# guanjq/targetdiff

Measured on NVIDIA H100. Metric: molecules/sec (1000-step sampling, CrossDocked pocket shape), higher is better.
Workload: dtype f32 (storage, LayerNorm, softmax, accumulation); GEMM operands as 2-piece bf16 splits on wgmma (3 products, ~16-bit operand mantissa)

## Files before the change

### targetdiff_b200/csrc/engine.cu

```cuda
#include <math.h>
#include <stdarg.h>
#include <stdio.h>
#include <stdlib.h>
#include <string.h>

#include <list>
#include <map>
#include <string>
#include <vector>

#include "../../include/tdiff.h"
#include "sampler.cuh"
#include "tdiff_common.cuh"

static thread_local char g_err[1024] = "";
static int set_err(int code, const char* fmt, ...) {
  va_list ap;
  va_start(ap, fmt);
  vsnprintf(g_err, sizeof(g_err), fmt, ap);
  va_end(ap);
  return code;
}
#define CK(call)                                                                                       \
  do {                                                                                                 \
// ... 36 lines not shown
  unsigned char* img_arena = nullptr;
  int mlp_mode = 2;
  bool mlp_v4 = true;
  std::vector<TdLayer> layers;
  const float *w_prot = nullptr, *b_prot = nullptr, *wl_t = nullptr, *bl = nullptr;
  const float *ew_w1t = nullptr, *ew_b1 = nullptr, *ew_g = nullptr, *ew_b = nullptr, *ew_w2 = nullptr, *ew_off = nullptr;
  float ew_b2 = 0.f, ew_coeff = -0.5f;
  int num_blocks = 1, ew_mode = 0 , out_fc = 0, time_emb = 0;
  int num_x2h = 1, num_h2x = 1, sync_twoup = 0;
  const float* w_time = nullptr;
  const float* zeros128 = nullptr;
  DevBuf ew_x2h, ew_h2x, hagg, time_norm;
  DevBuf h_sync;
  const float *hd_w1t = nullptr, *hd_b1 = nullptr, *hd_w2 = nullptr, *hd_b2 = nullptr;
  const float *t_c0 = nullptr, *t_ct = nullptr, *t_logvar = nullptr, *t_la = nullptr, *t_l1ma = nullptr, *t_lca = nullptr, *t_l1mca = nullptr,
              *t_sra = nullptr, *t_srm1 = nullptr;
  bool bound = false, has_ligand = false, have_graph = false;
  bool restrict_last = false;
  bool knn_incremental = false;
  bool have_prev = false;
  bool env_no_fused_agg = false, env_no_restrict = false, env_no_graph = false, env_knn_full = false, env_no_slot_keep = false;
  int B = 0, N = 0, Np = 0, Nl = 0, K = 0, max_ng = 0, final_buf = 0;
  int KQ = 0, hybrid = 0;
  DevBuf node_ptr, prot_ptr, prot_node, prot_graph, lig_node, lig_graph, node_lig;
  DevBuf rel_flag, rel_list, n_rel, work_list, n_work, knn_cache;
  DevBuf x2h_rows, lig_rows, rel_rows, rel_counts;
  long long x2h_n_dst = 0, x2h_split = 0, lig_n_dst = 0;
  int row_pad = 4;
  int free_depth = 0;
  int env_free_depth = 2;
  bool free_ready = false;
  DevBuf h_free, dirty, free_rows, free_counts, lig_save;
  long long free_stride = 0;
  DevBuf xm0, xm1, offset, h0, h, P, q, src, src_prev, etype, e_w, dist, kbuf, vbuf, v16, lig_pos, lig_v, logits;
  DevBuf step, err_flag, node_off, total_edges;
  DevBuf stage[8];
  cudaStream_t own_stream = nullptr;
  cudaEvent_t ev_fork = nullptr, ev_join = nullptr;
  long long launches = 0;
  bool profiling = false;
  std::vector<EvPair> events;
  double ms_acc[EV_KINDS] = {0, 0, 0, 0};
  long long n_acc[EV_KINDS] = {0, 0, 0, 0};
};

namespace {
struct Packer {
  std::map<std::string, const tdiff_tensor*> byname;
  std::vector<float> host;
  std::vector<unsigned char> img;
  std::string missing;
  std::list<std::vector<float>> keep;
  const float* get(const std::string& name, int64_t numel) {
    auto it = byname.find(name);
    if (it == byname.end() || it->second->numel != numel || it->second->data == nullptr) {
      if (missing.empty()) missing = name + (it == byname.end() ? " (absent)" : " (wrong size)");
      return nullptr;
    }
    return it->second->data;
  }
  size_t alloc(size_t n) {
    size_t off = (host.size() + 63) / 64 * 64;
    host.resize(off + n, 0.0f);
    return off;
  }
};
// ... 387 lines not shown
      const SubOff& so = is_h2x ? sh[l][idx - num_x2h] : sx[l][idx];
      sl.wn_t = A + so.wn_t; sl.bn = A + so.bn; sl.wn_img = IM ? IM + so.wn_img : nullptr;
      sl.k = mk_mlp(A, IM, so.k, 0, 256); sl.v = mk_mlp(A, IM, so.v, 128, 384); sl.q = mk_mlp(A, IM, so.q, 512, 512);
      sl.ew_w = so.ew_w >= 0 ? A + so.ew_w : nullptr; sl.ew_b = so.ew_b;
      sl.out_wa_img = so.out_wa >= 0 ? IM + so.out_wa : nullptr; sl.out_wb_img = so.out_wb >= 0 ? IM + so.out_wb : nullptr;
      sl.out_b1 = so.out_b1 >= 0 ? A + so.out_b1 : nullptr;
      memset(&sl.out, 0, sizeof(sl.out));
      if (so.out_w2 >= 0) {
        sl.out.w2_img = IM + so.out_w2; sl.out.ln_g = A + so.out_g; sl.out.ln_b = A + so.out_b; sl.out.b2 = A + so.out_b2; sl.out.nout = TD_H;
      }
    }
  }
  if (e->step.ensure(sizeof(int)) || e->err_flag.ensure(sizeof(int)) || e->total_edges.ensure(sizeof(long long))) {
    tdiff_destroy(e); return set_err(TDIFF_ECUDA, "cudaMalloc failed");
  }
  cudaMemset(e->err_flag.p, 0, sizeof(int));
  if (cudaStreamCreateWithFlags(&e->own_stream, cudaStreamNonBlocking) != cudaSuccess ||
      cudaEventCreateWithFlags(&e->ev_fork, cudaEventDisableTiming) != cudaSuccess ||
      cudaEventCreateWithFlags(&e->ev_join, cudaEventDisableTiming) != cudaSuccess) {
    tdiff_destroy(e); return set_err(TDIFF_ECUDA, "stream/event creation failed");
  }
  *out = e;
  return TDIFF_OK;
}

extern "C" void tdiff_destroy(tdiff_engine* e) {
  if (!e) return;
  cudaSetDevice(e->device);
  for (auto& ev : e->events) { cudaEventDestroy(ev.a); cudaEventDestroy(ev.b); }
  if (e->own_stream) cudaStreamDestroy(e->own_stream);
  if (e->ev_fork) cudaEventDestroy(e->ev_fork);
  if (e->ev_join) cudaEventDestroy(e->ev_join);
  DevBuf* bufs[] = {&e->node_ptr, &e->prot_ptr, &e->prot_node, &e->prot_graph, &e->lig_node, &e->lig_graph, &e->node_lig, &e->xm0, &e->xm1,
                    &e->rel_flag, &e->rel_list, &e->n_rel, &e->work_list, &e->n_work, &e->knn_cache, &e->x2h_rows, &e->lig_rows, &e->rel_rows, &e->rel_counts, &e->ew_x2h, &e->ew_h2x, &e->h_sync, &e->hagg, &e->time_norm, &e->h_free, &e->dirty, &e->free_rows, &e->free_counts, &e->lig_save, &e->offset, &e->h0, &e->h, &e->P, &e->q, &e->src, &e->src_prev, &e->etype, &e->e_w, &e->dist, &e->kbuf, &e->vbuf, &e->v16, &e->lig_pos,
                    &e->lig_v, &e->logits, &e->step, &e->err_flag, &e->node_off, &e->total_edges};
  for (auto* b : bufs) b->release();
  for (auto& b : e->stage) b.release();
  if (e->arena) cudaFree(e->arena);
  if (e->img_arena) cudaFree(e->img_arena);
  delete e;
}

extern "C" int tdiff_bind_batch(tdiff_engine* e, int B, const int32_t* pc, const int32_t* lc, const float* d_ppos, const float* d_pfeat,
                                int center_mode, void* stream) {
  if (!e || !pc || !lc || B < 1) return set_err(TDIFF_EINVAL, "bind_batch: bad arguments");
  if (center_mode != 0 && center_mode != 1) return set_err(TDIFF_EINVAL, "center_mode %d (0 'none' | 1 'protein')", center_mode);
  cudaStream_t st = (cudaStream_t)stream;
  CK(cudaSetDevice(e->device));
  long long N = 0, Np = 0, Nl = 0;
  int max_ng = 0;
  for (int g = 0; g < B; ++g) {
    if (pc[g] < 0 || lc[g] < 0) return set_err(TDIFF_EINVAL, "negative atom count in graph %d", g);
    Np += pc[g]; Nl += lc[g];
    if (pc[g] + lc[g] > max_ng) max_ng = pc[g] + lc[g];
  }
  N = Np + Nl;
  if (N <= 0) return set_err(TDIFF_EINVAL, "empty batch");
  if (e->hybrid) {
    int max_lc = 0;
    for (int g = 0; g < B; ++g) {
      if (lc[g] > max_lc) max_lc = lc[g];
      if (lc[g] > 0 && pc[g] < e->KQ)
        return set_err(TDIFF_EINVAL, "cutoff_mode 'hybrid': graph %d has %d protein atoms < k = %d (torch.topk fails in the reference too)", g, pc[g], e->KQ);
    }
    const int need = e->KQ + (max_lc > 0 ? max_lc - 1 : 0);
    if (need > TD_KMAX)
      return set_err(TDIFF_EINVAL, "cutoff_mode 'hybrid': k + n_ligand - 1 = %d + %d - 1 exceeds the %d neighbour slots per node", e->KQ, max_lc, TD_KMAX);
// ... 18 lines not shown
  bad |= e->node_ptr.ensure((B + 1) * 4) | e->prot_ptr.ensure((B + 1) * 4) | e->prot_node.ensure(Np * 4 + 4) | e->prot_graph.ensure(Np * 4 + 4);
  bad |= e->lig_node.ensure(Nl * 4 + 4) | e->lig_graph.ensure(Nl * 4 + 4) | e->node_lig.ensure(N * 4);
  bad |= e->xm0.ensure(N * 16) | e->xm1.ensure(N * 16) | e->offset.ensure((size_t)B * 16);
  bad |= e->h0.ensure(N * TD_H * 4) | e->h.ensure(N * TD_H * 4) | e->P.ensure((size_t)(N + 1) * TD_NPROJ * 4) | e->q.ensure(N * TD_H * 4);
  bad |= e->src.ensure(slots * 4) | e->src_prev.ensure(slots * 4) | e->etype.ensure(slots) | e->e_w.ensure(slots * 4) | e->dist.ensure(slots * 4);
  const bool v4 = e->mlp_mode == 2 && e->mlp_v4;
  int gcd128 = 128;
  while (K % gcd128) gcd128 >>= 1;
  e->row_pad = 128 / gcd128;
  const long long pad = e->row_pad, nPpad = (Np + pad - 1) / pad * pad, nLpad = (Nl + pad - 1) / pad * pad;
  e->x2h_n_dst = nPpad + nLpad; e->x2h_split = nPpad; e->lig_n_dst = nLpad;
  std::vector<int> x2h_rows((size_t)(nPpad + nLpad), -1), lig_rows((size_t)nLpad, -1);
  for (long long i = 0; i < Np; ++i) x2h_rows[i] = prot_node[i];
  for (long long i = 0; i < Nl; ++i) { x2h_rows[nPpad + i] = lig_node[i]; lig_rows[i] = lig_node[i]; }
  if (v4) bad |= e->x2h_rows.ensure(x2h_rows.size() * 4 + 4) | e->lig_rows.ensure(lig_rows.size() * 4 + 4) | e->rel_rows.ensure(x2h_rows.size() * 4 + 4) |
                 e->rel_counts.ensure(16);
  const bool fuse = v4 && K == 32 && !e->env_no_fused_agg && e->ew_mode != 2;
  if (e->ew_mode == 1) bad |= e->ew_x2h.ensure(slots * 4) | e->ew_h2x.ensure(slots * 4);
  if (e->out_fc) bad |= e->hagg.ensure((size_t)N * TD_H * 4);
  if (e->sync_twoup && e->num_x2h > 0 && e->num_h2x > 0) bad |= e->h_sync.ensure((size_t)N * TD_H * 4);
  if (e->time_emb) bad |= e->time_norm.ensure((size_t)B * 4 + 16);
  bad |= e->kbuf.ensure(v4 ? (size_t)(nPpad + nLpad) * K * TD_HEADS * 4 + 64 : slots * TD_H * 4);
  if (!fuse) bad |= e->vbuf.ensure(slots * TD_H * 4);
  bad |= e->v16.ensure((size_t)nLpad * K * TD_HEADS * 4 + 16);
  int min_pc = 1 << 30;
  for (int g = 0; g < B; ++g) if (pc[g] < min_pc) min_pc = pc[g];
  e->free_ready = false;
  e->free_depth = (fuse && !e->hybrid && Nl > 0 && min_pc > K) ? e->env_free_depth : 0;
  const int x2h_evals = (int)e->layers.size() * e->num_x2h;
  if (e->free_depth > x2h_evals - 1) e->free_depth = x2h_evals - 1 > 0 ? x2h_evals - 1 : 0;
  if (e->free_depth > 0)
    bad |= e->h_free.ensure((size_t)e->free_depth * N * TD_H * 4) | e->dirty.ensure((size_t)e->free_depth * N + 16) |
           e->free_rows.ensure((size_t)e->free_depth * x2h_rows.size() * 4 + 4) | e->free_counts.ensure((size_t)e->free_depth * 16) |
           e->lig_save.ensure((size_t)Nl * 20 + 32);
  e->free_stride = (long long)x2h_rows.size();
  bad |= e->lig_pos.ensure(Nl * 16 + 16) | e->lig_v.ensure(Nl * 4 + 4) | e->logits.ensure((size_t)Nl * e->cfg.num_classes * 4 + 4);
  bad |= e->node_off.ensure(N * 8) | e->rel_flag.ensure(N + 16) | e->rel_list.ensure(N * 4 + 64) | e->n_rel.ensure(16) | e->work_list.ensure(N * 4 + 64) | e->n_work.ensure(16);
  e->knn_incremental = !e->env_knn_full && Np > 0;
  if (e->knn_incremental) bad |= e->knn_cache.ensure((size_t)N * (e->KQ + 1) * 8);
  if (bad) return set_err(TDIFF_ECUDA, "out of device memory binding a batch of %lld nodes (%zu edge slots)", N, slots);
  CK(cudaMemcpyAsync(e->node_ptr.p, node_ptr.data(), (B + 1) * 4, cudaMemcpyHostToDevice, st));
  CK(cudaMemcpyAsync(e->prot_ptr.p, prot_ptr.data(), (B + 1) * 4, cudaMemcpyHostToDevice, st));
  if (Np) {
    CK(cudaMemcpyAsync(e->prot_node.p, prot_node.data(), Np * 4, cudaMemcpyHostToDevice, st));
    CK(cudaMemcpyAsync(e->prot_graph.p, prot_graph.data(), Np * 4, cudaMemcpyHostToDevice, st));
  }
  if (Nl) {
    CK(cudaMemcpyAsync(e->lig_node.p, lig_node.data(), Nl * 4, cudaMemcpyHostToDevice, st));
    CK(cudaMemcpyAsync(e->lig_graph.p, lig_graph.data(), Nl * 4, cudaMemcpyHostToDevice, st));
  }
  CK(cudaMemcpyAsync(e->node_lig.p, node_lig.data(), N * 4, cudaMemcpyHostToDevice, st));
  if (v4) {
    if (!x2h_rows.empty()) CK(cudaMemcpyAsync(e->x2h_rows.p, x2h_rows.data(), x2h_rows.size() * 4, cudaMemcpyHostToDevice, st));
    if (!lig_rows.empty()) CK(cudaMemcpyAsync(e->lig_rows.p, lig_rows.data(), lig_rows.size() * 4, cudaMemcpyHostToDevice, st));
  }
  CK(cudaStreamSynchronize(st));
  CK(cudaMemsetAsync(e->offset.p, 0, (size_t)B * 16, st));
  if (e->time_emb) CK(cudaMemsetAsync(e->time_norm.p, 0, (size_t)B * 4, st));
  CK(cudaMemsetAsync(e->h0.p, 0, (size_t)N * TD_H * 4, st));
  CK(cudaMemsetAsync(e->xm0.p, 0, (size_t)N * 16, st));
  CK(cudaMemsetAsync(e->xm1.p, 0, (size_t)N * 16, st));
  CK(cudaMemsetAsync(e->etype.p, 0, slots, st));
  CK(cudaMemsetAsync(e->P.as<float>() + (size_t)N * TD_NPROJ, 0, (size_t)TD_NPROJ * 4, st));
  if (center_mode == 1) td_launch_segment_mean3(d_ppos, e->prot_ptr.as<int>(), B, e->offset.as<float4>(), st);
  td_launch_place_protein(d_ppos, e->prot_node.as<int>(), e->prot_graph.as<int>(), e->offset.as<float4>(), (int)Np, e->xm0.as<float4>(),
                          e->xm1.as<float4>(), st);
  td_launch_protein_embed(d_pfeat, (int)Np, e->cfg.protein_feat_dim, e->w_prot, e->b_prot, e->prot_node.as<int>(), e->h0.as<float>(), st);
  e->launches += 3;
  if (e->knn_incremental) {
    td_launch_knn_cache(e->xm0.as<float4>(), e->node_ptr.as<int>(), e->prot_ptr.as<int>(), B, max_ng, e->KQ, e->knn_cache.as<unsigned long long>(), st);
    e->launches += 1;
  }
  CK(cudaGetLastError());
  e->bound = true;
  return TDIFF_OK;
}

extern "C" int tdiff_set_ligand(tdiff_engine* e, const float* d_pos, const int64_t* d_v, int apply_center, void* stream) {
  if (!e || !e->bound) return set_err(TDIFF_ESTATE, "set_ligand before bind_batch");
  if (e->Nl > 0 && !d_pos) return set_err(TDIFF_EINVAL, "null ligand positions");
  if (!e->has_ligand && e->Nl > 0 && !d_v) return set_err(TDIFF_EINVAL, "ligand types required on first set_ligand");
  cudaStream_t st = (cudaStream_t)stream;
  CK(cudaSetDevice(e->device));
  td_launch_set_ligand(d_pos, (const long long*)d_v, e->lig_graph.as<int>(), e->offset.as<float4>(), apply_center, e->Nl,
                       e->cfg.num_classes, e->lig_pos.as<float4>(), e->lig_v.as<int>(), e->err_flag.as<int>(), st);
  e->launches += 1;
  if (d_v) {
    int flag = 0;
    CK(cudaMemcpyAsync(&flag, e->err_flag.p, sizeof(int), cudaMemcpyDeviceToHost, st));
    CK(cudaStreamSynchronize(st));
    if (flag) {
      cudaMemsetAsync(e->err_flag.p, 0, sizeof(int), st);
      e->has_ligand = false;
      return set_err(TDIFF_EINVAL, "ligand atom type index >= num_classes (%d)", e->cfg.num_classes);
    }
  }
// ... 29 lines not shown
  }
  ~Prof() { if (on) { cudaEventRecord(ev.b, st); e->events.push_back(ev); } }
};

enum RowList { ROWS_ALL = 0, ROWS_LIGAND = 1, ROWS_RELEVANT = 2 };
bool fused_logits(const tdiff_engine* e) { return e->mlp_mode == 2 && e->mlp_v4; }
void edge_mlp(tdiff_engine* e, const float* P, const float4* xm, const int* src, const unsigned char* etype, RowList list, int K, const TdMlp& m,
              const float* offsets, float coeff, float* out, cudaStream_t st, const float* e_w, const float* qnode = nullptr,
              const float* agg_logits = nullptr, float* agg_h = nullptr, int key_softmax = 0, int free_layer = -1) {
  if (fused_logits(e) && m.w2_img && m.tabcls_img) {
    const int* rows = list == ROWS_ALL ? e->x2h_rows.as<int>() : list == ROWS_LIGAND ? e->lig_rows.as<int>() : e->rel_rows.as<int>();
    const int* counts = list == ROWS_RELEVANT ? e->rel_counts.as<int>() : nullptr;
    if (free_layer >= 0) {
      rows = e->free_rows.as<int>() + (size_t)free_layer * e->free_stride;
      counts = e->free_counts.as<int>() + 4 * free_layer;
    }
    const long long n_dst = list == ROWS_LIGAND ? e->lig_n_dst : e->x2h_n_dst;
    const long long split = list == ROWS_LIGAND ? 0 : e->x2h_split;
    const int by_slot = (list != ROWS_LIGAND && !key_softmax && agg_logits == nullptr) ? 1 : 0;
    td_launch_edge_mlp_v4(P, e->N, src, etype, e->dist.as<float>(), rows, n_dst, split, counts, K, m,
                          e->host_arena.data() + (offsets - e->arena), coeff, e->host_arena.data() + (m.ln_b - e->arena),
                          e->host_arena.data() + (m.b2 - e->arena), qnode, out, by_slot, agg_logits, e_w, agg_h, key_softmax,
                          e->sm_count, st);
    return;
  }
  const int* row_nodes = list == ROWS_LIGAND ? e->lig_node.as<int>() : nullptr;
  const long long n_rows = (long long)(list == ROWS_LIGAND ? e->Nl : e->N) * K;
  if (e->mlp_mode != 0 && m.nout == TD_H && m.w2_img)
    td_launch_edge_mlp_tc(P, xm, src, etype, e->dist.as<float>(), row_nodes, n_rows, K, m, m.w2_img, e->mlp_mode, offsets, coeff, out, e->sm_count, st);
  else
    td_launch_edge_mlp(P, xm, src, etype, row_nodes, n_rows, K, m, offsets, coeff, out, e->sm_count, st);
}

void node_side(tdiff_engine* e, const float* h, int N, const TdSubLayer& sl, float* P, float* q, cudaStream_t st, const int* rows = nullptr,
               const int* d_n = nullptr) {
  if (fused_logits(e) && sl.wn_img && sl.q.w2_img) {
    td_launch_node_side_v4(h, N, sl.wn_img, sl.bn, sl.q, P, q, rows, d_n, e->sm_count, st);
  } else if (e->mlp_mode != 0 && sl.wn_img && sl.q.w2_img) {
    TdMlp pm = sl.q;
    pm.b2 = sl.bn;
    td_launch_rows_tc(1, h, TD_H, 0, N, pm, sl.wn_img, e->mlp_mode, P, TD_NPROJ, TD_NPROJ / TD_H, rows, d_n, e->sm_count, st);
    td_launch_rows_tc(2, P, TD_NPROJ, 512, N, sl.q, sl.q.w2_img, e->mlp_mode, q, TD_H, 1, rows, d_n, e->sm_count, st);
  } else {
    td_launch_node_proj(h, N, sl.wn_t, sl.bn, P, st);
    td_launch_node_q(P, N, sl.q, q, st);
  }
}

void run_forward(tdiff_engine* e, cudaStream_t st, int fix_x, int free_build = 0, float* blk_pos = nullptr, float* blk_logits = nullptr) {
  const int N = e->N, Nl = e->Nl, K = e->K;
  float4* xm[2] = {e->xm0.as<float4>(), e->xm1.as<float4>()};
  const int* src = e->src.as<int>();
  const unsigned char* etype = e->etype.as<unsigned char>();
  float* h = e->h.as<float>();
  float* P = e->P.as<float>();
  float* q = e->q.as<float>();
  td_launch_scatter_ligand_pos(e->lig_pos.as<float4>(), e->lig_node.as<int>(), Nl, xm[0], st);
  td_launch_init_h(e->h0.as<float>(), xm[0], e->lig_v.as<int>(), e->node_lig.as<int>(), e->wl_t, e->bl, e->w_time, e->time_norm.as<float>(),
                   e->lig_graph.as<int>(), N, h, st);
  e->launches += 2;
  int cur = 0;
  const int KC = e->cfg.num_classes;
  auto snapshot = [&](int i) {
    if (blk_pos) {
      td_launch_gather_xyz(xm[cur], e->lig_node.as<int>(), Nl, blk_pos + (size_t)i * Nl * 3, st);
      e->launches += 1;
    }
    if (blk_logits) {
      td_launch_head(h, e->lig_node.as<int>(), Nl, e->hd_w1t, e->hd_b1, e->hd_w2, e->hd_b2, KC, blk_logits + (size_t)i * Nl * KC, st);
      e->launches += 1;
    }
  };
  if (Nl > 0) snapshot(0);
  const int n_blocks = free_build ? 1 : e->num_blocks;
  for (int blk = 0; blk < n_blocks; ++blk) {
// ... 9 lines not shown
                         use_free ? e->dirty.as<unsigned char>() : nullptr, e->work_list.as<int>(), e->n_work.as<int>(), (e->ew_mode != 0 ? 1 : 0) | (e->env_no_slot_keep ? 2 : 0), st);
    e->have_prev = true;
    for (int l = 0; l < use_free; ++l) {
      unsigned char* dl = e->dirty.as<unsigned char>() + (size_t)l * N;
      if (l > 0) td_launch_dirty_propagate(dl - N, src, N, K, dl, st);
      td_launch_rel_rows(dl, xm[cur], N, e->lig_rows.as<int>(), (int)e->lig_n_dst, e->row_pad, e->free_rows.as<int>() + (size_t)l * e->free_stride,
                         e->free_counts.as<int>() + 4 * l, st);
      e->launches += l > 0 ? 3 : 2;
    }
    td_launch_rel_compact(e->rel_flag.as<unsigned char>(), N, e->rel_list.as<int>(), e->n_rel.as<int>(), st);
    e->launches += 4;
    if (fused_logits(e) && e->restrict_last && last_blk && e->num_x2h > 0) {
      td_launch_rel_rows(e->rel_flag.as<unsigned char>(), xm[cur], N, e->lig_rows.as<int>(), (int)e->lig_n_dst, e->row_pad, e->rel_rows.as<int>(),
                         e->rel_counts.as<int>(), st);
      e->launches += 2;
    }
    const float4* xm_blk = xm[cur];
    const int NX = e->num_x2h, NH = e->num_h2x;
    const size_t L = e->layers.size();
    int g = 0;
    for (size_t l = 0; l < L && !(free_build && g >= free_build); ++l) {
      const TdLayer& ly = e->layers[l];
      const float* ew_x = e->ew_mode == 1 ? e->ew_x2h.as<float>() : e->e_w.as<float>();
      const float* ew_h = e->ew_mode == 1 ? e->ew_h2x.as<float>() : e->e_w.as<float>();
      const bool run_h2x = !free_build && !fix_x && Nl > 0 && NH > 0;
      const float* h_h2x = h;
      if (e->sync_twoup && run_h2x && NX > 0) {
        cudaMemcpyAsync(e->h_sync.p, h, (size_t)N * TD_H * 4, cudaMemcpyDeviceToDevice, st);
        h_h2x = e->h_sync.as<float>();
      }
      for (int i = 0; i < NX && !(free_build && g >= free_build); ++i, ++g) {
        const TdSubLayer& sx = ly.x2h[i];
        const int fl = g < use_free ? g : -1;
        node_side(e, h, N, sx, P, q, st);
        if (e->mlp_mode != 0 && (i == 0 || e->ew_mode == 1)) {
          TdEwR ew = {nullptr, nullptr, 0.f, 0.f, ly.offsets, ly.coeff, nullptr, nullptr};
          if (e->ew_mode == 1) {
            const TdSubLayer& sh0 = NH > 0 ? ly.h2x[0] : sx;
            ew.w_x2h = sx.ew_w; ew.w_h2x = sh0.ew_w; ew.b_x2h = sx.ew_b; ew.b_h2x = sh0.ew_b; ew.out_x2h = e->ew_x2h.as<float>(); ew.out_h2x = e->ew_h2x.as<float>();
          }
          td_launch_edge_geom(xm[cur], src, etype, N, K, e->dist.as<float>(), ew, st);
          e->launches += 1;
        }
        const bool fuse_agg = fused_logits(e) && K == 32 && !e->env_no_fused_agg && e->ew_mode != 2;
        const bool sub = fuse_agg && e->restrict_last && last_blk && l + 1 == L && i + 1 == NX && !e->env_no_restrict && !e->out_fc;
        const RowList rl = sub ? ROWS_RELEVANT : ROWS_ALL;
        float* agg_target = h;
        if (e->out_fc) {
          agg_target = e->hagg.as<float>();
          cudaMemsetAsync(agg_target, 0, (size_t)N * TD_H * 4, st);
        }
        {
          Prof pr(e, st, EV_EDGE_MLP);
          edge_mlp(e, P, xm[cur], src, etype, rl, K, sx.k, ly.offsets, ly.coeff, e->kbuf.as<float>(), st, ew_x, fused_logits(e) ? q : nullptr, nullptr,
                   nullptr, fuse_agg ? 1 : 0, fl);
          edge_mlp(e, P, xm[cur], src, etype, rl, K, sx.v, ly.offsets, ly.coeff, e->vbuf.as<float>(), st, ew_x, nullptr,
                   fuse_agg ? e->kbuf.as<float>() : nullptr, fuse_agg ? agg_target : nullptr, 0, fl);
        }
        if (!fuse_agg) {
          Prof pr(e, st, EV_AGG_H);
          if (fused_logits(e))
            td_launch_aggregate_h_logits(e->kbuf.as<float>(), e->vbuf.as<float>(), ew_x, src, e->out_fc ? agg_target : h, agg_target, N, K,
                                         e->ew_mode == 2 ? sx.ew_w : nullptr, sx.ew_b, st);
          else td_launch_aggregate_h(e->kbuf.as<float>(), e->vbuf.as<float>(), e->e_w.as<float>(), src, q, h, h, N, K, st);
        }
        e->launches += fuse_agg ? 4 : 5;
        if (e->out_fc) {
          float* t1 = P;
          float* t2 = P + (size_t)N * TD_H;
          TdMlp m1 = sx.out;
          m1.b2 = e->zeros128;
          td_launch_rows_tc(1, agg_target, TD_H, 0, N, m1, sx.out_wa_img, e->mlp_mode, t1, TD_H, 1, nullptr, nullptr, e->sm_count, st);
          m1.b2 = sx.out_b1;
          td_launch_rows_tc(1, h, TD_H, 0, N, m1, sx.out_wb_img, e->mlp_mode, t2, TD_H, 1, nullptr, nullptr, e->sm_count, st);
          td_launch_add_rows(t1, t2, t1, (long long)N * TD_H, st);
          td_launch_rows_tc(2, t1, TD_H, 0, N, sx.out, sx.out.w2_img, e->mlp_mode, t2, TD_H, 1, nullptr, nullptr, e->sm_count, st);
          td_launch_add_rows(h, t2, h, (long long)N * TD_H, st);
          e->launches += 6;
        }
        if (fl >= 0) {
          td_launch_restore_clean(e->dirty.as<unsigned char>() + (size_t)fl * N, xm_blk, e->h_free.as<float>() + (size_t)fl * N * TD_H, N, h, st);
          e->launches += 1;
        }
        if (free_build) cudaMemcpyAsync(e->h_free.as<float>() + (size_t)g * N * TD_H, h, (size_t)N * TD_H * 4, cudaMemcpyDeviceToDevice, st);
      }
      if (!run_h2x) continue;
      for (int j = 0; j < NH; ++j) {
        const TdSubLayer& sh = ly.h2x[j];
        if (j > 0 || NX == 0) {
          td_launch_edge_geom_rows(xm[cur], src, etype, e->lig_node.as<int>(), Nl, K, e->dist.as<float>(), e->ew_mode == 1 ? sh.ew_w : nullptr, sh.ew_b,
                                   ly.offsets, ly.coeff, e->ew_h2x.as<float>(), st);
          e->launches += 1;
        }
        {
          const bool rel = fused_logits(e) && !e->env_no_restrict;
          node_side(e, h_h2x, N, sh, P, q, st, rel ? e->rel_list.as<int>() : nullptr, rel ? e->n_rel.as<int>() : nullptr);
        }
        {
          Prof pr(e, st, EV_EDGE_MLP);
          edge_mlp(e, P, xm[cur], src, etype, ROWS_LIGAND, K, sh.k, ly.offsets, ly.coeff, e->kbuf.as<float>(), st, ew_h, fused_logits(e) ? q : nullptr);
          edge_mlp(e, P, xm[cur], src, etype, ROWS_LIGAND, K, sh.v, ly.offsets, ly.coeff, e->v16.as<float>(), st, ew_h);
        }
        {
          Prof pr(e, st, EV_AGG_X);
          if (fused_logits(e))
            td_launch_aggregate_x_logits(e->kbuf.as<float>(), e->v16.as<float>(), ew_h, src, xm[cur], e->lig_node.as<int>(), xm[cur ^ 1], Nl, K, st);
          else
            td_launch_aggregate_x(e->kbuf.as<float>(), e->v16.as<float>(), e->e_w.as<float>(), src, q, xm[cur], e->lig_node.as<int>(), xm[cur ^ 1], Nl, K, st);
        }
        e->launches += 5;
        cur ^= 1;
      }
    }
    if (Nl > 0) snapshot(blk + 1);
  }
  if (free_build) return;
  td_launch_head(h, e->lig_node.as<int>(), Nl, e->hd_w1t, e->hd_b1, e->hd_w2, e->hd_b2, e->cfg.num_classes, e->logits.as<float>(), st);
  e->launches += 1;
  e->final_buf = cur;
  e->have_graph = true;
  e->have_prev = true;
}
}

extern "C" int tdiff_set_time(tdiff_engine* e, const float* d_time_norm, void* stream) {
  if (!e || !e->bound) return set_err(TDIFF_ESTATE, "set_time before bind_batch");
  if (!e->time_emb) return TDIFF_OK;
  if (!d_time_norm) return set_err(TDIFF_EINVAL, "null time array");
  CK(cudaSetDevice(e->device));
  CK(cudaMemcpyAsync(e->time_norm.p, d_time_norm, (size_t)e->B * 4, cudaMemcpyDeviceToDevice, (cudaStream_t)stream));
// ... 367 lines not shown
```

### targetdiff_b200/csrc/node_side.cu

```cuda
#include "tdiff_common.cuh"
#include "hopper_mma.cuh"

namespace ns {

constexpr int kWG = 3;
constexpr int kThreads = kWG * 128;
constexpr int kTile = 64;
constexpr int kAtom = 128 * 128;
constexpr int kPiece = 2 * kAtom;
constexpr int kBlock = 2 * kPiece;
constexpr int kImgStride = 3 * kPiece;
constexpr int kHBuf = kTile * TD_H * 4;
constexpr size_t kSmem = 1024 + 2 * kBlock + kWG * kHBuf + 4 * TD_H * sizeof(float);
static_assert(kSmem <= 227 * 1024, "shared-memory map");

__device__ __forceinline__ uint32_t smem_u32(const void* p) { return (uint32_t)__cvta_generic_to_shared(p); }
__device__ __forceinline__ uint32_t cvt_bf16x2(float hi, float lo) {
  uint32_t d;
  asm("cvt.rn.bf16x2.f32 %0, %1, %2;" : "=r"(d) : "f"(hi), "f"(lo));
  return d;
}
__device__ __forceinline__ void stg64(float* p, float a, float b) { asm volatile("st.global.v2.f32 [%0], {%1,%2};" ::"l"(p), "f"(a), "f"(b) : "memory"); }
__device__ __forceinline__ void fence_proxy_async() { asm volatile("fence.proxy.async.shared::cta;" ::: "memory"); }

__device__ __forceinline__ void stage_weights(unsigned char* sW, const unsigned char* w0, const unsigned char* w1, float* sPar,
                                              const float* p0, const float* p1, const float* p2, const float* p3) {
  for (int i = threadIdx.x; i < kBlock / 16; i += kThreads) {
    reinterpret_cast<uint4*>(sW)[i] = reinterpret_cast<const uint4*>(w0)[i];
    reinterpret_cast<uint4*>(sW + kBlock)[i] = reinterpret_cast<const uint4*>(w1)[i];
  }
  for (int i = threadIdx.x; i < TD_H; i += kThreads) {
    if (p0) sPar[i] = p0[i];
    if (p1) sPar[TD_H + i] = p1[i];
    if (p2) sPar[2 * TD_H + i] = p2[i];
    if (p3) sPar[3 * TD_H + i] = p3[i];
  }
  fence_proxy_async();
  __syncthreads();
}

struct Rows {
  const int* list;
  const int* d_n;
  long long n;
};

__device__ __forceinline__ uint32_t chunk_pos(int r, int c) { return (uint32_t)(r * 512 + ((c ^ ((r & 3) << 1)) << 4)); }
__device__ __forceinline__ void bar_sync_wg(int wg) { asm volatile("bar.sync %0, 128;" ::"r"(1 + wg) : "memory"); }

__device__ __forceinline__ void load_tile_async(uint32_t buf, const float* __restrict__ in, const Rows& rw, long long n, long long tile, int t) {
  const int l = t & 31;
#pragma unroll 1
  for (int r = t >> 5; r < kTile; r += 4) {
    const long long i = tile * kTile + r;
    const long long node = i < n ? (rw.list ? (long long)rw.list[i] : i) : 0;
    asm volatile("cp.async.cg.shared.global [%0], [%1], 16, %2;" ::"r"(buf + chunk_pos(r, l)), "l"(in + (size_t)node * TD_H + 4 * l),
                 "r"(i < n ? 16 : 0) : "memory");
  }
  asm volatile("cp.async.commit_group;" ::: "memory");
}

__device__ __forceinline__ void read_tile(uint32_t buf, int w, int l, float (&x)[64]) {
  const int s = (l >> 2) & 3;
  const uint32_t base = buf + (uint32_t)(16 * w + (l >> 2)) * 512 + ((l & 3) >> 1) * 16 + (l & 1) * 8;
#pragma unroll
  for (int j = 0; j < 4; ++j) {
    const uint32_t p = base + ((j ^ s) << 5);
#pragma unroll
    for (int hh = 0; hh < 2; ++hh)
#pragma unroll
      for (int I = 0; I < 4; ++I) {
        const int i = 4 * I + j;
        float2 v;
        asm volatile("ld.shared.v2.f32 {%0, %1}, [%2];" : "=f"(v.x), "=f"(v.y) : "r"(p + hh * 8 * 512 + I * 128));
        x[4 * i + 2 * hh] = v.x;
        x[4 * i + 2 * hh + 1] = v.y;
      }
  }
}

__device__ __forceinline__ void split_frag(const float (&x)[64], uint32_t (&a)[2][8][4]) {
#pragma unroll
  for (int kk = 0; kk < 8; ++kk)
#pragma unroll
    for (int j = 0; j < 4; ++j) {
      const int e = 4 * (2 * kk + (j >> 1)) + 2 * (j & 1);
      const float x0 = x[e], x1 = x[e + 1];
      const uint32_t v = cvt_bf16x2(x1, x0);
      a[0][kk][j] = v;
// ... 19 lines not shown
#pragma unroll
  for (int hh = 0; hh < 2; ++hh) {
    if (prow[hh] < 0) continue;
    float* o = out + (size_t)prow[hh] * ldo + col0;
#pragma unroll
    for (int i = 0; i < 16; ++i) {
      const int c = 8 * i + 2 * (l & 3);
      stg64(o + c, d[4 * i + 2 * hh] + sBias[c], d[4 * i + 2 * hh + 1] + sBias[c + 1]);
    }
  }
}

__device__ __forceinline__ void next_tile(uint32_t buf, const float* __restrict__ in, const Rows& rw, long long n, long long next, int wg, int t,
                                          float (&x)[64]) {
  asm volatile("cp.async.wait_all;" ::: "memory");
  bar_sync_wg(wg);
  read_tile(buf, t >> 5, t & 31, x);
  bar_sync_wg(wg);
  if (next >= 0) load_tile_async(buf, in, rw, n, next, t);
}

__device__ __forceinline__ void tile_rows(const Rows& rw, long long n, long long tile, int w, int l, int (&prow)[2]) {
#pragma unroll
  for (int hh = 0; hh < 2; ++hh) {
    const long long i = tile * kTile + 16 * w + (l >> 2) + 8 * hh;
    prow[hh] = i < n ? (rw.list ? rw.list[i] : (int)i) : -1;
  }
}

}

__global__ void __launch_bounds__(ns::kThreads, 1)
node_proj_kernel(const float* __restrict__ h, const unsigned char* __restrict__ wn_img, const float* __restrict__ bn, float* __restrict__ P,
                 ns::Rows rw) {
  using namespace ns;
  extern __shared__ unsigned char smem_raw[];
  unsigned char* sW = reinterpret_cast<unsigned char*>((reinterpret_cast<uintptr_t>(smem_raw) + 1023) & ~(uintptr_t)1023);
  float* sBias = reinterpret_cast<float*>(sW + 2 * kBlock + kWG * kHBuf);
  const int g = blockIdx.y;
  const long long n = rw.d_n ? (long long)*rw.d_n : rw.n;
  const long long n_tiles = (n + kTile - 1) / kTile, stride = (long long)gridDim.x * kWG;
  const int t = threadIdx.x & 127, l = t & 31, w = t >> 5;
  const int wg = __shfl_sync(0xffffffffu, threadIdx.x >> 7, 0);
  const uint32_t buf = smem_u32(sW + 2 * kBlock) + wg * kHBuf, w_addr = smem_u32(sW);
  long long tile = blockIdx.x * kWG + wg;
  if (tile < n_tiles) load_tile_async(buf, h, rw, n, tile, t);
  stage_weights(sW, wn_img + (size_t)(2 * g) * kImgStride, wn_img + (size_t)(2 * g + 1) * kImgStride, sBias, bn + 256 * g, bn + 256 * g + 128,
                nullptr, nullptr);
#pragma unroll 1
  for (; tile < n_tiles; tile += stride) {
    int prow[2];
    tile_rows(rw, n, tile, w, l, prow);
    uint32_t a[2][8][4];
    {
      float x[64];
      next_tile(buf, h, rw, n, tile + stride < n_tiles ? tile + stride : -1, wg, t, x);
      split_frag(x, a);
    }
#pragma unroll 1
    for (int j = 0; j < 2; ++j) {
      float d[64];
      mma_block(d, a, w_addr + j * kBlock);
      store_rows(P, TD_NPROJ, 256 * g + 128 * j, prow, l, d, sBias + 128 * j);
    }
  }
}

__global__ void __launch_bounds__(ns::kThreads, 1)
node_query_kernel(const float* __restrict__ h, const unsigned char* __restrict__ wq_img, const float* __restrict__ bq, TdMlp m,
                  float* __restrict__ q, ns::Rows rw) {
  using namespace ns;
  extern __shared__ unsigned char smem_raw[];
  unsigned char* sW = reinterpret_cast<unsigned char*>((reinterpret_cast<uintptr_t>(smem_raw) + 1023) & ~(uintptr_t)1023);
  float* sBq = reinterpret_cast<float*>(sW + 2 * kBlock + kWG * kHBuf);
  float* sG = sBq + TD_H;
  float* sB = sG + TD_H;
  float* sB2 = sB + TD_H;
  const long long n = rw.d_n ? (long long)*rw.d_n : rw.n;
// ... 20 lines not shown
        d[4 * i + 2 * hh] += sBq[c];
        d[4 * i + 2 * hh + 1] += sBq[c + 1];
        s += d[4 * i + 2 * hh] + d[4 * i + 2 * hh + 1];
      }
      s += __shfl_xor_sync(0xffffffffu, s, 1);
      s += __shfl_xor_sync(0xffffffffu, s, 2);
      const float mean = s * (1.0f / 128.0f);
      float v = 0.f;
#pragma unroll
      for (int i = 0; i < 16; ++i) {
        const float e0 = d[4 * i + 2 * hh] - mean, e1 = d[4 * i + 2 * hh + 1] - mean;
        d[4 * i + 2 * hh] = e0;
        d[4 * i + 2 * hh + 1] = e1;
        v += e0 * e0 + e1 * e1;
      }
      v += __shfl_xor_sync(0xffffffffu, v, 1);
      v += __shfl_xor_sync(0xffffffffu, v, 2);
      const float rstd = 1.0f / sqrtf(v * (1.0f / 128.0f) + 1e-5f);
#pragma unroll
      for (int i = 0; i < 16; ++i) {
        const int c = 8 * i + 2 * (l & 3);
        d[4 * i + 2 * hh] = fmaxf(d[4 * i + 2 * hh] * rstd * sG[c] + sB[c], 0.f);
        d[4 * i + 2 * hh + 1] = fmaxf(d[4 * i + 2 * hh + 1] * rstd * sG[c + 1] + sB[c + 1], 0.f);
      }
    }
    split_frag(d, a);
    mma_block(d, a, w_addr + kBlock);
    int prow[2];
    tile_rows(rw, n, tile, w, l, prow);
    store_rows(q, TD_H, 0, prow, l, d, sB2);
  }
}

void td_launch_node_side_v4(const float* h, long long n_rows, const unsigned char* wn_img, const float* bn, const TdMlp& q_mlp, float* P,
                            float* q, const int* rows, const int* d_n, int sm_count, cudaStream_t st) {
  using namespace ns;
  if (n_rows == 0) return;
  static size_t opted_p[TD_MAX_DEVICES] = {0}, opted_q[TD_MAX_DEVICES] = {0};
  td_opt_in_smem(node_proj_kernel, kSmem, opted_p);
  td_opt_in_smem(node_query_kernel, kSmem, opted_q);
  const Rows rw = {rows, d_n, n_rows};
  const long long slots = (n_rows + kTile - 1) / kTile;
  const long long ctas = (slots + kWG - 1) / kWG;
  const int per = sm_count / 2 > 0 ? sm_count / 2 : 1;
  node_proj_kernel<<<dim3((unsigned)(ctas < per ? ctas : per), 2), kThreads, kSmem, st>>>(h, wn_img, bn, P, rw);
  node_query_kernel<<<(unsigned)(ctas < sm_count ? ctas : sm_count), kThreads, kSmem, st>>>(h, wn_img + 4 * (size_t)kImgStride, bn + 512, q_mlp,
                                                                                           q, rw);
}
```

### targetdiff_b200/csrc/tdiff_common.cuh

```cuda
#pragma once
#include <cuda_runtime.h>
#include <stdint.h>

#define TD_H 128
#define TD_HEADS 16
#define TD_HD 8
#define TD_NG 20
#define TD_TAB 21
#define TD_KMAX 64
#define TD_NPROJ 640
#define TD_CMAX 24

struct TdMlp {
  const float* tab;
  const float* ln_g;
  const float* ln_b;
  const float* w2t;
  const float* b2;
  int nout;
  int offA, offB;
  const unsigned char* w2_img;
  const unsigned char* tabcls_img;
};

// ... 93 lines not shown
                         cudaStream_t st);
void td_launch_knn_update(const float4* xm, const int* node_ptr, const int* prot_ptr, int n_graphs, int max_ng, int k, int stride, int hybrid,
                          const unsigned long long* cache, int* src, cudaStream_t st);
void td_launch_edge_const(const float4* xm, const int* src, int* src_prev, int have_prev, int n_nodes, int k, const float* offsets, float coeff,
                          const float* w1t, const float* b1, const float* ln_g, const float* ln_b, const float* w2, float b2,
                          unsigned char* etype, float* e_w, unsigned char* rel_flag, unsigned char* touch_flag, int* work_list, int* n_work,
                          int gate_mode, cudaStream_t st);
void td_launch_dirty_propagate(const unsigned char* in, const int* src, int n_nodes, int k, unsigned char* out, cudaStream_t st);
void td_launch_restore_clean(const unsigned char* dirty, const float4* xm, const float* h_free, int n_nodes, float* h, cudaStream_t st);
void td_launch_rel_rows(const unsigned char* rel_flag, const float4* xm, int n_nodes, const int* lig_rows, int n_lig_rows, int pad, int* rel_rows,
                        int* rel_counts, cudaStream_t st);
void td_launch_protein_embed(const float* feat, int n_protein, int fdim, const float* w, const float* b, const int* prot_node,
                             float* h0, cudaStream_t st);
void td_launch_init_h(const float* h0, const float4* xm, const int* lig_v, const int* node_lig, const float* wl_t, const float* bl,
                      const float* w_time, const float* time_norm, const int* lig_graph, int n_nodes, float* h, cudaStream_t st);
void td_launch_node_proj(const float* h, int n_nodes, const float* wn_t, const float* bn, float* P, cudaStream_t st);
void td_launch_node_q(const float* P, int n_nodes, TdMlp q, float* qout, cudaStream_t st);
void td_launch_edge_mlp(const float* P, const float4* xm, const int* src, const unsigned char* etype, const int* row_nodes,
                        long long n_rows, int k, TdMlp m, const float* offsets, float coeff, float* out, int sm_count, cudaStream_t st);
void td_launch_edge_geom(const float4* xm, const int* src, const unsigned char* etype, int n_nodes, int k, float* dist, const TdEwR& ew, cudaStream_t st);
void td_launch_edge_geom_rows(const float4* xm, const int* src, const unsigned char* etype, const int* rows, int n_rows, int k, float* dist,
                              const float* gate_w, float gate_b, const float* offsets, float coeff, float* gate, cudaStream_t st);
void td_launch_add_rows(const float* a, const float* b, float* out, long long n_floats, cudaStream_t st);
void td_launch_set_time(const int* step, int t_start, int n_timesteps, int n_graphs, float* time_norm, cudaStream_t st);
void td_launch_edge_mlp_tc(const float* P, const float4* xm, const int* src, const unsigned char* etype, const float* dist,
                           const int* row_nodes, long long n_rows, int k, TdMlp m, const unsigned char* w2_image, int pieces, const float* offsets, float coeff,
                           float* out, int sm_count, cudaStream_t st);
void td_launch_edge_mlp_v4(const float* P, int zero_row, const int* src, const unsigned char* etype, const float* dist, const int* row_nodes, long long n_dst,
                           long long split_dst, const int* d_counts, int k, const TdMlp& m, const float* h_offsets, float coeff,
                           const float* h_ln_b, const float* h_b2, const float* qnode, float* out, int out_by_slot,
                           const float* agg_logits, const float* agg_e_w, float* agg_h, int key_softmax, int sm_count, cudaStream_t st);
void td_launch_rows_tc(int mode, const float* in, int ldi, int in_off, long long n_rows, TdMlp m, const unsigned char* w_image, int pieces, float* out,
                       int ldo, int nblocks, const int* row_list, const int* d_n_rows, int sm_count, cudaStream_t st);
void td_launch_node_side_v4(const float* h, long long n_rows, const unsigned char* wn_img, const float* bn, const TdMlp& q_mlp, float* P,
                            float* q, const int* rows, const int* d_n, int sm_count, cudaStream_t st);
void td_launch_rel_compact(const unsigned char* flag, int n_nodes, int* rel_list, int* n_rel, cudaStream_t st);
void td_launch_aggregate_h(const float* kbuf, const float* vbuf, const float* e_w, const int* src, const float* q, const float* h_in,
                           float* h_out, int n_nodes, int k, cudaStream_t st);
void td_launch_aggregate_x(const float* kbuf, const float* v16, const float* e_w, const int* src, const float* q, const float4* xm_in,
                           const int* row_nodes, float4* xm_out, int n_rows, int k, cudaStream_t st);
void td_launch_aggregate_h_logits(const float* logits, const float* vbuf, const float* e_w, const int* src, const float* h_in, float* h_out,
                                  int n_nodes, int k, const float* ewm_w, float ewm_b, cudaStream_t st);
void td_launch_aggregate_x_logits(const float* logits, const float* v16, const float* e_w, const int* src, const float4* xm_in,
                                  const int* row_nodes, float4* xm_out, int n_rows, int k, cudaStream_t st);
void td_launch_head(const float* h, const int* lig_node, int n_lig, const float* w1t, const float* b1, const float* w2, const float* b2,
                    int n_classes, float* logits, cudaStream_t st);
void td_launch_check_stability(const float* pos, const int* atomic_num, const int* mol_ptr, int n_mol, int hs, int* nr_bonds, int* stable_atoms,
                               unsigned char* mol_stable, int* err, cudaStream_t st);
```

Before: 18.26.

## Split node projections into destination/source row sets and cache first-layer protein projections

The node-side projection kernel now takes separate destination and source row lists. The grid is partitioned so the query/destination half of P is computed only for the needed rows, such as ligand nodes, while the source half covers relevant rows. Projections for the first x2h sublayer go into persistent P0/q0 buffers, so later steps recompute only ligand rows and reuse the unchanged protein rows. Weight staging and row gathering also move to cp.async with shuffled row indices. This adds complexity and risks stale protein projections if the caching assumptions break.

```diff
diff --git a/targetdiff_b200/csrc/engine.cu b/targetdiff_b200/csrc/engine.cu
--- a/targetdiff_b200/csrc/engine.cu
+++ b/targetdiff_b200/csrc/engine.cu
@@ -92,6 +92,7 @@
   bool free_ready = false;
   DevBuf h_free, dirty, free_rows, free_counts, lig_save;
   long long free_stride = 0;
+  DevBuf P0, q0;
   DevBuf xm0, xm1, offset, h0, h, P, q, src, src_prev, etype, e_w, dist, kbuf, vbuf, v16, lig_pos, lig_v, logits;
   DevBuf step, err_flag, node_off, total_edges;
   DevBuf stage[8];
@@ -545,7 +546,7 @@
   if (e->ev_fork) cudaEventDestroy(e->ev_fork);
   if (e->ev_join) cudaEventDestroy(e->ev_join);
   DevBuf* bufs[] = {&e->node_ptr, &e->prot_ptr, &e->prot_node, &e->prot_graph, &e->lig_node, &e->lig_graph, &e->node_lig, &e->xm0, &e->xm1,
-                    &e->rel_flag, &e->rel_list, &e->n_rel, &e->work_list, &e->n_work, &e->knn_cache, &e->x2h_rows, &e->lig_rows, &e->rel_rows, &e->rel_counts, &e->ew_x2h, &e->ew_h2x, &e->h_sync, &e->hagg, &e->time_norm, &e->h_free, &e->dirty, &e->free_rows, &e->free_counts, &e->lig_save, &e->offset, &e->h0, &e->h, &e->P, &e->q, &e->src, &e->src_prev, &e->etype, &e->e_w, &e->dist, &e->kbuf, &e->vbuf, &e->v16, &e->lig_pos,
+                    &e->rel_flag, &e->rel_list, &e->n_rel, &e->work_list, &e->n_work, &e->knn_cache, &e->x2h_rows, &e->lig_rows, &e->rel_rows, &e->rel_counts, &e->ew_x2h, &e->ew_h2x, &e->h_sync, &e->hagg, &e->time_norm, &e->h_free, &e->dirty, &e->free_rows, &e->free_counts, &e->lig_save, &e->P0, &e->q0, &e->offset, &e->h0, &e->h, &e->P, &e->q, &e->src, &e->src_prev, &e->etype, &e->e_w, &e->dist, &e->kbuf, &e->vbuf, &e->v16, &e->lig_pos,
                     &e->lig_v, &e->logits, &e->step, &e->err_flag, &e->node_off, &e->total_edges};
   for (auto* b : bufs) b->release();
   for (auto& b : e->stage) b.release();
@@ -630,7 +631,7 @@
   if (e->free_depth > 0)
     bad |= e->h_free.ensure((size_t)e->free_depth * N * TD_H * 4) | e->dirty.ensure((size_t)e->free_depth * N + 16) |
            e->free_rows.ensure((size_t)e->free_depth * x2h_rows.size() * 4 + 4) | e->free_counts.ensure((size_t)e->free_depth * 16) |
-           e->lig_save.ensure((size_t)Nl * 20 + 32);
+           e->lig_save.ensure((size_t)Nl * 20 + 32) | e->P0.ensure((size_t)(N + 1) * TD_NPROJ * 4) | e->q0.ensure((size_t)N * TD_H * 4);
   e->free_stride = (long long)x2h_rows.size();
   bad |= e->lig_pos.ensure(Nl * 16 + 16) | e->lig_v.ensure(Nl * 4 + 4) | e->logits.ensure((size_t)Nl * e->cfg.num_classes * 4 + 4);
   bad |= e->node_off.ensure(N * 8) | e->rel_flag.ensure(N + 16) | e->rel_list.ensure(N * 4 + 64) | e->n_rel.ensure(16) | e->work_list.ensure(N * 4 + 64) | e->n_work.ensure(16);
@@ -660,6 +661,7 @@
   CK(cudaMemsetAsync(e->xm1.p, 0, (size_t)N * 16, st));
   CK(cudaMemsetAsync(e->etype.p, 0, slots, st));
   CK(cudaMemsetAsync(e->P.as<float>() + (size_t)N * TD_NPROJ, 0, (size_t)TD_NPROJ * 4, st));
+  if (e->free_depth > 0) CK(cudaMemsetAsync(e->P0.as<float>() + (size_t)N * TD_NPROJ, 0, (size_t)TD_NPROJ * 4, st));
   if (center_mode == 1) td_launch_segment_mean3(d_ppos, e->prot_ptr.as<int>(), B, e->offset.as<float4>(), st);
   td_launch_place_protein(d_ppos, e->prot_node.as<int>(), e->prot_graph.as<int>(), e->offset.as<float4>(), (int)Np, e->xm0.as<float4>(),
                           e->xm1.as<float4>(), st);
@@ -755,15 +757,17 @@
     td_launch_edge_mlp(P, xm, src, etype, row_nodes, n_rows, K, m, offsets, coeff, out, e->sm_count, st);
 }
 
-void node_side(tdiff_engine* e, const float* h, int N, const TdSubLayer& sl, float* P, float* q, cudaStream_t st, const int* rows = nullptr,
-               const int* d_n = nullptr) {
+struct NodeRows { const int* list = nullptr; const int* d_n = nullptr; long long n = -1; };
+void node_side(tdiff_engine* e, const float* h, int N, const TdSubLayer& sl, float* P, float* q, cudaStream_t st, NodeRows dst = {},
+               NodeRows src = {}) {
   if (fused_logits(e) && sl.wn_img && sl.q.w2_img) {
-    td_launch_node_side_v4(h, N, sl.wn_img, sl.bn, sl.q, P, q, rows, d_n, e->sm_count, st);
+    td_launch_node_side_v4(h, dst.n < 0 ? N : dst.n, dst.list, dst.d_n, src.n < 0 ? N : src.n, src.list, src.d_n, sl.wn_img, sl.bn, sl.q, P, q,
+                           e->sm_count, st);
   } else if (e->mlp_mode != 0 && sl.wn_img && sl.q.w2_img) {
     TdMlp pm = sl.q;
     pm.b2 = sl.bn;
-    td_launch_rows_tc(1, h, TD_H, 0, N, pm, sl.wn_img, e->mlp_mode, P, TD_NPROJ, TD_NPROJ / TD_H, rows, d_n, e->sm_count, st);
-    td_launch_rows_tc(2, P, TD_NPROJ, 512, N, sl.q, sl.q.w2_img, e->mlp_mode, q, TD_H, 1, rows, d_n, e->sm_count, st);
+    td_launch_rows_tc(1, h, TD_H, 0, N, pm, sl.wn_img, e->mlp_mode, P, TD_NPROJ, TD_NPROJ / TD_H, nullptr, nullptr, e->sm_count, st);
+    td_launch_rows_tc(2, P, TD_NPROJ, 512, N, sl.q, sl.q.w2_img, e->mlp_mode, q, TD_H, 1, nullptr, nullptr, e->sm_count, st);
   } else {
     td_launch_node_proj(h, N, sl.wn_t, sl.bn, P, st);
     td_launch_node_q(P, N, sl.q, q, st);
@@ -839,7 +843,20 @@
       for (int i = 0; i < NX && !(free_build && g >= free_build); ++i, ++g) {
         const TdSubLayer& sx = ly.x2h[i];
         const int fl = g < use_free ? g : -1;
-        node_side(e, h, N, sx, P, q, st);
+        const bool fuse_agg = fused_logits(e) && K == 32 && !e->env_no_fused_agg && e->ew_mode != 2;
+        const bool sub = fuse_agg && e->restrict_last && last_blk && l + 1 == L && i + 1 == NX && !e->env_no_restrict && !e->out_fc;
+        const RowList rl = sub ? ROWS_RELEVANT : ROWS_ALL;
+        const bool first0 = g == 0 && (free_build || use_free > 0);
+        float* Px = first0 ? e->P0.as<float>() : P;
+        float* qx = first0 ? e->q0.as<float>() : q;
+        if (first0 && !free_build) {
+          const NodeRows lig = {e->lig_node.as<int>(), nullptr, Nl};
+          node_side(e, h, N, sx, Px, qx, st, lig, lig);
+        } else if (sub) {
+          node_side(e, h, N, sx, Px, qx, st, NodeRows{e->rel_list.as<int>(), e->n_rel.as<int>(), N});
+        } else {
+          node_side(e, h, N, sx, Px, qx, st);
+        }
         if (e->mlp_mode != 0 && (i == 0 || e->ew_mode == 1)) {
           TdEwR ew = {nullptr, nullptr, 0.f, 0.f, ly.offsets, ly.coeff, nullptr, nullptr};
           if (e->ew_mode == 1) {
@@ -849,9 +866,6 @@
           td_launch_edge_geom(xm[cur], src, etype, N, K, e->dist.as<float>(), ew, st);
           e->launches += 1;
         }
-        const bool fuse_agg = fused_logits(e) && K == 32 && !e->env_no_fused_agg && e->ew_mode != 2;
-        const bool sub = fuse_agg && e->restrict_last && last_blk && l + 1 == L && i + 1 == NX && !e->env_no_restrict && !e->out_fc;
-        const RowList rl = sub ? ROWS_RELEVANT : ROWS_ALL;
         float* agg_target = h;
         if (e->out_fc) {
           agg_target = e->hagg.as<float>();
@@ -859,9 +873,9 @@
         }
         {
           Prof pr(e, st, EV_EDGE_MLP);
-          edge_mlp(e, P, xm[cur], src, etype, rl, K, sx.k, ly.offsets, ly.coeff, e->kbuf.as<float>(), st, ew_x, fused_logits(e) ? q : nullptr, nullptr,
+          edge_mlp(e, Px, xm[cur], src, etype, rl, K, sx.k, ly.offsets, ly.coeff, e->kbuf.as<float>(), st, ew_x, fused_logits(e) ? qx : nullptr, nullptr,
                    nullptr, fuse_agg ? 1 : 0, fl);
-          edge_mlp(e, P, xm[cur], src, etype, rl, K, sx.v, ly.offsets, ly.coeff, e->vbuf.as<float>(), st, ew_x, nullptr,
+          edge_mlp(e, Px, xm[cur], src, etype, rl, K, sx.v, ly.offsets, ly.coeff, e->vbuf.as<float>(), st, ew_x, nullptr,
                    fuse_agg ? e->kbuf.as<float>() : nullptr, fuse_agg ? agg_target : nullptr, 0, fl);
         }
         if (!fuse_agg) {
@@ -899,10 +913,10 @@
                                    ly.offsets, ly.coeff, e->ew_h2x.as<float>(), st);
           e->launches += 1;
         }
-        {
-          const bool rel = fused_logits(e) && !e->env_no_restrict;
-          node_side(e, h_h2x, N, sh, P, q, st, rel ? e->rel_list.as<int>() : nullptr, rel ? e->n_rel.as<int>() : nullptr);
-        }
+        if (fused_logits(e) && !e->env_no_restrict)
+          node_side(e, h_h2x, N, sh, P, q, st, NodeRows{e->lig_node.as<int>(), nullptr, Nl}, NodeRows{e->rel_list.as<int>(), e->n_rel.as<int>(), N});
+        else
+          node_side(e, h_h2x, N, sh, P, q, st);
         {
           Prof pr(e, st, EV_EDGE_MLP);
           edge_mlp(e, P, xm[cur], src, etype, ROWS_LIGAND, K, sh.k, ly.offsets, ly.coeff, e->kbuf.as<float>(), st, ew_h, fused_logits(e) ? q : nullptr);
diff --git a/targetdiff_b200/csrc/node_side.cu b/targetdiff_b200/csrc/node_side.cu
--- a/targetdiff_b200/csrc/node_side.cu
+++ b/targetdiff_b200/csrc/node_side.cu
@@ -25,16 +25,19 @@
 
 __device__ __forceinline__ void stage_weights(unsigned char* sW, const unsigned char* w0, const unsigned char* w1, float* sPar,
                                               const float* p0, const float* p1, const float* p2, const float* p3) {
+  const uint32_t s0 = (uint32_t)__cvta_generic_to_shared(sW), s1 = s0 + kBlock;
   for (int i = threadIdx.x; i < kBlock / 16; i += kThreads) {
-    reinterpret_cast<uint4*>(sW)[i] = reinterpret_cast<const uint4*>(w0)[i];
-    reinterpret_cast<uint4*>(sW + kBlock)[i] = reinterpret_cast<const uint4*>(w1)[i];
-  }
+    asm volatile("cp.async.cg.shared.global [%0], [%1], 16;" ::"r"(s0 + 16 * i), "l"(w0 + 16 * (size_t)i) : "memory");
+    asm volatile("cp.async.cg.shared.global [%0], [%1], 16;" ::"r"(s1 + 16 * i), "l"(w1 + 16 * (size_t)i) : "memory");
+  }
+  asm volatile("cp.async.commit_group;" ::: "memory");
   for (int i = threadIdx.x; i < TD_H; i += kThreads) {
     if (p0) sPar[i] = p0[i];
     if (p1) sPar[TD_H + i] = p1[i];
     if (p2) sPar[2 * TD_H + i] = p2[i];
     if (p3) sPar[3 * TD_H + i] = p3[i];
   }
+  asm volatile("cp.async.wait_all;" ::: "memory");
   fence_proxy_async();
   __syncthreads();
 }
@@ -49,12 +52,15 @@
 __device__ __forceinline__ void bar_sync_wg(int wg) { asm volatile("bar.sync %0, 128;" ::"r"(1 + wg) : "memory"); }
 
 __device__ __forceinline__ void load_tile_async(uint32_t buf, const float* __restrict__ in, const Rows& rw, long long n, long long tile, int t) {
-  const int l = t & 31;
-#pragma unroll 1
-  for (int r = t >> 5; r < kTile; r += 4) {
-    const long long i = tile * kTile + r;
-    const long long node = i < n ? (rw.list ? (long long)rw.list[i] : i) : 0;
-    asm volatile("cp.async.cg.shared.global [%0], [%1], 16, %2;" ::"r"(buf + chunk_pos(r, l)), "l"(in + (size_t)node * TD_H + 4 * l),
+  const int l = t & 31, w = t >> 5;
+  const long long i0 = tile * kTile + w;
+  const long long il = i0 + 4 * (l & 15);
+  const int my_node = il < n ? (rw.list ? rw.list[il] : (int)il) : 0;
+#pragma unroll 4
+  for (int j = 0; j < kTile / 4; ++j) {
+    const long long i = i0 + 4 * j;
+    const int node = __shfl_sync(0xffffffffu, my_node, j);
+    asm volatile("cp.async.cg.shared.global [%0], [%1], 16, %2;" ::"r"(buf + chunk_pos(w + 4 * j, l)), "l"(in + (size_t)node * TD_H + 4 * l),
                  "r"(i < n ? 16 : 0) : "memory");
   }
   asm volatile("cp.async.commit_group;" ::: "memory");
@@ -140,18 +146,25 @@
 
 __global__ void __launch_bounds__(ns::kThreads, 1)
 node_proj_kernel(const float* __restrict__ h, const unsigned char* __restrict__ wn_img, const float* __restrict__ bn, float* __restrict__ P,
-                 ns::Rows rw) {
+                 ns::Rows rd, ns::Rows rs) {
   using namespace ns;
   extern __shared__ unsigned char smem_raw[];
   unsigned char* sW = reinterpret_cast<unsigned char*>((reinterpret_cast<uintptr_t>(smem_raw) + 1023) & ~(uintptr_t)1023);
   float* sBias = reinterpret_cast<float*>(sW + 2 * kBlock + kWG * kHBuf);
-  const int g = blockIdx.y;
-  const long long n = rw.d_n ? (long long)*rw.d_n : rw.n;
-  const long long n_tiles = (n + kTile - 1) / kTile, stride = (long long)gridDim.x * kWG;
+  const long long nd = rd.d_n ? (long long)*rd.d_n : rd.n, ns_ = rs.d_n ? (long long)*rs.d_n : rs.n;
+  const long long td = (nd + kTile - 1) / kTile, ts = (ns_ + kTile - 1) / kTile;
+  const int G = (int)gridDim.x;
+  int c0 = td + ts > 0 ? (int)(((long long)G * td + (td + ts) / 2) / (td + ts)) : 0;
+  if (ts > 0 && c0 > G - 1) c0 = G - 1;
+  if (td > 0 && c0 < 1) c0 = 1;
+  const int g = (int)blockIdx.x < c0 ? 0 : 1;
+  const Rows rw = g ? rs : rd;
+  const long long n = g ? ns_ : nd;
+  const long long n_tiles = g ? ts : td, stride = (long long)(g ? G - c0 : c0) * kWG;
   const int t = threadIdx.x & 127, l = t & 31, w = t >> 5;
   const int wg = __shfl_sync(0xffffffffu, threadIdx.x >> 7, 0);
   const uint32_t buf = smem_u32(sW + 2 * kBlock) + wg * kHBuf, w_addr = smem_u32(sW);
-  long long tile = blockIdx.x * kWG + wg;
+  long long tile = (long long)((int)blockIdx.x - (g ? c0 : 0)) * kWG + wg;
   if (tile < n_tiles) load_tile_async(buf, h, rw, n, tile, t);
   stage_weights(sW, wn_img + (size_t)(2 * g) * kImgStride, wn_img + (size_t)(2 * g + 1) * kImgStride, sBias, bn + 256 * g, bn + 256 * g + 128,
                 nullptr, nullptr);
@@ -238,18 +251,20 @@
   }
 }
 
-void td_launch_node_side_v4(const float* h, long long n_rows, const unsigned char* wn_img, const float* bn, const TdMlp& q_mlp, float* P,
-                            float* q, const int* rows, const int* d_n, int sm_count, cudaStream_t st) {
+void td_launch_node_side_v4(const float* h, long long n_dst, const int* dst_rows, const int* dst_n, long long n_src, const int* src_rows,
+                            const int* src_n, const unsigned char* wn_img, const float* bn, const TdMlp& q_mlp, float* P, float* q, int sm_count,
+                            cudaStream_t st) {
   using namespace ns;
-  if (n_rows == 0) return;
+  if (n_dst == 0 && n_src == 0) return;
   static size_t opted_p[TD_MAX_DEVICES] = {0}, opted_q[TD_MAX_DEVICES] = {0};
   td_opt_in_smem(node_proj_kernel, kSmem, opted_p);
   td_opt_in_smem(node_query_kernel, kSmem, opted_q);
-  const Rows rw = {rows, d_n, n_rows};
-  const long long slots = (n_rows + kTile - 1) / kTile;
-  const long long ctas = (slots + kWG - 1) / kWG;
+  const Rows rd = {dst_rows, dst_n, n_dst}, rs = {src_rows, src_n, n_src};
+  auto ctas_for = [](long long n) { return ((n + kTile - 1) / kTile + kWG - 1) / kWG; };
+  const long long cd = ctas_for(n_dst), cs = ctas_for(n_src);
   const int per = sm_count / 2 > 0 ? sm_count / 2 : 1;
-  node_proj_kernel<<<dim3((unsigned)(ctas < per ? ctas : per), 2), kThreads, kSmem, st>>>(h, wn_img, bn, P, rw);
-  node_query_kernel<<<(unsigned)(ctas < sm_count ? ctas : sm_count), kThreads, kSmem, st>>>(h, wn_img + 4 * (size_t)kImgStride, bn + 512, q_mlp,
-                                                                                           q, rw);
-}
+  node_proj_kernel<<<(unsigned)(cd + cs < 2 * per ? cd + cs : 2 * per), kThreads, kSmem, st>>>(h, wn_img, bn, P, rd, rs);
+  if (n_dst > 0)
+    node_query_kernel<<<(unsigned)(cd < sm_count ? cd : sm_count), kThreads, kSmem, st>>>(h, wn_img + 4 * (size_t)kImgStride, bn + 512, q_mlp,
+                                                                                         q, rd);
+}
diff --git a/targetdiff_b200/csrc/tdiff_common.cuh b/targetdiff_b200/csrc/tdiff_common.cuh
--- a/targetdiff_b200/csrc/tdiff_common.cuh
+++ b/targetdiff_b200/csrc/tdiff_common.cuh
@@ -149,8 +149,9 @@
                            const float* agg_logits, const float* agg_e_w, float* agg_h, int key_softmax, int sm_count, cudaStream_t st);
 void td_launch_rows_tc(int mode, const float* in, int ldi, int in_off, long long n_rows, TdMlp m, const unsigned char* w_image, int pieces, float* out,
                        int ldo, int nblocks, const int* row_list, const int* d_n_rows, int sm_count, cudaStream_t st);
-void td_launch_node_side_v4(const float* h, long long n_rows, const unsigned char* wn_img, const float* bn, const TdMlp& q_mlp, float* P,
-                            float* q, const int* rows, const int* d_n, int sm_count, cudaStream_t st);
+void td_launch_node_side_v4(const float* h, long long n_dst, const int* dst_rows, const int* dst_n, long long n_src, const int* src_rows,
+                            const int* src_n, const unsigned char* wn_img, const float* bn, const TdMlp& q_mlp, float* P, float* q, int sm_count,
+                            cudaStream_t st);
 void td_launch_rel_compact(const unsigned char* flag, int n_nodes, int* rel_list, int* n_rel, cudaStream_t st);
 void td_launch_aggregate_h(const float* kbuf, const float* vbuf, const float* e_w, const int* src, const float* q, const float* h_in,
                            float* h_out, int n_nodes, int k, cudaStream_t st);
```

New measurement: 18.79 (median of 6 runs). 1.03x the previous value.
